# fnothaft/spark-bam

Hardware: AMD Instinct MI355X
Metric: compressed BAM GB/s for compute-splits + full-check (whole node, 1/2/4/8 GPU) (higher is better)
Workload: dtype u8

## Files before the change

### spark-bam_amd/csrc/sbam_api.cpp

```cpp
#include "../../include/sbam.h"

#include <algorithm>
#include <cstdarg>
#include <cstdio>
#include <cstdlib>
#include <cstring>
#include <map>
#include <string>
#include <vector>

#include "sbam_deflate_core.h"
#include "sbam_internal.h"
#include "sbam_layout.h"
#include "sbam_tag_core.h"

using namespace sbam;
using namespace sbam_layout;

namespace {

#define HIPTRY(expr)                 \
  do {                               \
    hipError_t e_ = (expr);          \
    if (e_ != hipSuccess) return e_; \
// ... 184 lines not shown
  DevBuf<int64_t> d_tokbase;
  DevBuf<int32_t> d_slow;
  DevBuf<unsigned int> d_icnt;
  int64_t inflate_slow = -1;
  DevBuf<uint32_t> d_crc, d_crcst;
  int64_t crc_b0 = -1, crc_b1 = -1;
  bool verify_crc = false;
  int32_t nref = -1;
  DevBuf<int64_t> d_lens;
  std::vector<int64_t> h_lens;
  sbam_pos header_end{0, 0, 0};
  int64_t header_x = -1;
  DevBuf<unsigned long long> d_bitmap;
  int64_t bm_x0 = 0, bm_x1 = 0;
  int32_t bm_R = -1;
  bool bm_valid = false;
  bool bm_list = false;
  int64_t plist_n = 0;
  DevBuf<int32_t> d_ccnt;
  DevBuf<int32_t> d_tcnt;
  DevBuf<int64_t> d_coff2, d_plist, d_pfb;
  DevBuf<uint8_t> d_pok;
  DevBuf<unsigned long long> d_nfb;
  DevBuf<int64_t> d_sx, d_se, d_sn, d_sb;
  int32_t rp_tried = 0, rp_proved = 0;
  int64_t rp_missing = -1, rp_failed = -1;
  bool rp_fetch = false;
  DevBuf<int64_t> d_roff;
  DevBuf<uint8_t> d_rcols;
  RecordColumnsDev rcols{};
  int64_t n_loaded = -1;
  DevBuf<uint8_t> d_foff, d_fdata;
  sbam_record_fields fdev{};
  int64_t f_i0 = 0, f_n = -1;
  sbam_record_field_totals f_tot{};
  DevBuf<uint8_t> d_tcell, d_toff, d_tdata;
  sbam_record_tags tdev{};
  int64_t t_i0 = 0, t_n = -1;
  int32_t t_nq = 0;
  bool t_bytes[SBAM_MAX_TAGS] = {};
  sbam_record_tag_totals t_tot{};
  bool loaded_all = false;
  DevBuf<int32_t> d_iend;
  DevBuf<uint32_t> d_ibin;
  DevBuf<int64_t> d_iheads, d_iintv;
  DevBuf<uint8_t> d_istat;
// ... 17 lines not shown
  std::string path = "<bytes>";
};

namespace {

int set_err(sbam_ctx *c, int code, const char *fmt, ...) {
  c->err.code = code;
  va_list ap;
  va_start(ap, fmt);
  vsnprintf(c->err.message, sizeof(c->err.message), fmt, ap);
  va_end(ap);
  return code;
}

#define HIPCHK(ctx, expr)                                                                     \
  do {                                                                                        \
    hipError_t e_ = (expr);                                                                   \
    if (e_ != hipSuccess) return set_err(ctx, SBAM_ERR_HIP, "%s: %s", #expr, hipGetErrorString(e_)); \
  } while (0)

struct Timer {
  sbam_ctx *c;
  std::pair<hipEvent_t, hipEvent_t> *e = nullptr;
  Timer(sbam_ctx *c_, const char *name) : c(c_) {
    if (!c) return;
    auto it = c->ev.find(name);
    if (it == c->ev.end()) {
      std::pair<hipEvent_t, hipEvent_t> p;
      (void)hipEventCreate(&p.first);
      (void)hipEventCreate(&p.second);
      it = c->ev.emplace(name, p).first;
    }
    e = &it->second;
    (void)hipEventRecord(e->first, c->stream);
  }
  ~Timer() { if (c) (void)hipEventRecord(e->second, c->stream); }
};

#define SMALL(c, word) ((c)->d_small.get() + offsetof(Scratch, word) / 8)
#define USMALL(c, word) reinterpret_cast<unsigned long long *>(SMALL(c, word))

template <class F>
hipError_t carve(DevBuf<uint8_t> &buf, bool *grew, F &&layout) {
  Carve size(nullptr);
  layout(size);
  HIPTRY(buf.ensure(size.bytes(), grew));
  Carve k(buf.get());
  layout(k);
  return hipSuccess;
}

StreamView view(sbam_ctx *c) {
  return StreamView{c->d_u, c->L, c->d_lens, c->nref, (c->base + c->D >= c->file_size) ? 1 : 0};
}

void set_bitmap(sbam_ctx *c, int64_t x0, int64_t x1, int32_t R, bool list_form) {
  c->bm_x0 = x0 & ~(int64_t)63;
  c->bm_x1 = x1;
  c->bm_R = R;
// ... 225 lines not shown
  c->file_size = file_size;
  HIPCHK(c, hipSetDevice(device));
  HIPCHK(c, hipStreamCreateWithFlags(&c->stream, hipStreamNonBlocking));
  HIPCHK(c, c->d_comp.ensure((size_t)len + kCompPad));
  HIPCHK(c, hipMemsetAsync(c->d_comp + len, 0, kCompPad, c->stream));
  if (len) HIPCHK(c, hipMemcpyAsync(c->d_comp, data, (size_t)len, hipMemcpyHostToDevice, c->stream));
  HIPCHK(c, c->d_small.ensure(sizeof(Scratch) / 8));
  HIPCHK(c, carve(c->d_counts, nullptr, count_words<CountsDev>));
  HIPCHK(c, hipStreamSynchronize(c->stream));
  return SBAM_OK;
}

void sbam_close(sbam_ctx *c) {
  if (!c) return;
  (void)hipSetDevice(c->device);
  if (c->stream) (void)hipStreamSynchronize(c->stream);
  if (c->blk.copy_stream) (void)hipStreamSynchronize(c->blk.copy_stream);
  for (auto &kv : c->ev) {
    (void)hipEventDestroy(kv.second.first);
    (void)hipEventDestroy(kv.second.second);
  }
  for (hipEvent_t e : c->load_ev)
    if (e) (void)hipEventDestroy(e);
  c->blk.destroy();
  if (c->stream) (void)hipStreamDestroy(c->stream);
  delete c;
}

const sbam_error *sbam_last_error(const sbam_ctx *c) { return c ? &c->err : nullptr; }

int sbam_set_path(sbam_ctx *c, const char *path) {
  if (!c || !path) return SBAM_ERR_ARG;
  c->path = path;
  return SBAM_OK;
}

int sbam_load(sbam_ctx *c, const uint8_t *data, int64_t len, int64_t base_offset, int64_t file_size) {
  if (!c || (!data && len > 0) || len < 0 || base_offset < 0 || file_size < base_offset + len) return SBAM_ERR_ARG;
  HIPCHK(c, hipSetDevice(c->device));
  HIPCHK(c, hipStreamSynchronize(c->stream));
  HIPCHK(c, c->d_comp.ensure((size_t)len + kCompPad));
  HIPCHK(c, hipMemsetAsync(c->d_comp + len, 0, kCompPad, c->stream));
  constexpr int64_t kPiece = 8ll << 20;
  constexpr int kInFlight = 3;
  for (hipEvent_t &e : c->load_ev)
    if (!e) HIPCHK(c, hipEventCreateWithFlags(&e, hipEventDisableTiming));
// ... 31 lines not shown
  HIPCHK(c, ensure_inflate(c, ubytes, n_blocks, &grew));
  HIPCHK(c, ensure_check(c, 0, ubytes, &grew));
  if (n_records > 0) {
    const size_t n = (size_t)(n_records + n_records / 8 + 4096);
    HIPCHK(c, ensure_chain_list(c, n, &grew));
    HIPCHK(c, ensure_record_columns(c, n, &grew));
  }
  if (grew && any_stage_ran(c)) return sbam_reset(c);
  return SBAM_OK;
}

int sbam_reset(sbam_ctx *c) {
  if (!c) return SBAM_ERR_ARG;
  const hipError_t e = drop_from(c, kCandidates);
  c->err = sbam_error{};
  HIPCHK(c, e);
  return SBAM_OK;
}

double sbam_last_kernel_ms(sbam_ctx *c, const char *kernel) {
  if (!std::strcmp(kernel, "record_tags")) {
    const double walk = sbam_last_kernel_ms(c, "record_tag_walk"), bytes = sbam_last_kernel_ms(c, "record_tag_bytes");
    return walk < 0 ? -1.0 : walk + (bytes < 0 ? 0.0 : bytes);
  }
  auto it = c->ev.find(kernel);
  if (it == c->ev.end()) return -1.0;
  (void)hipEventSynchronize(it->second.second);
  float ms = -1.f;
  if (hipEventElapsedTime(&ms, it->second.first, it->second.second) != hipSuccess) return -1.0;
  return ms;
}

static int scan_candidates(sbam_ctx *c) {
  if (c->ncand >= 0) return SBAM_OK;
  Timer t(c, "scan");
  const int64_t nchunks = scan_chunks(c->D);
  HIPCHK(c, ensure_scan(c, c->D));
  HIPCHK(c, launch_scan_slots(c->d_comp, c->D, c->d_cc, nchunks, c->d_slots, SMALL(c, scan_overflow), c->stream));
  HIPCHK(c, launch_scan_sums(c->d_cc, c->d_coff, nchunks, 1, SMALL(c, scan_total), c->stream));
  int64_t tot_ovf[2] = {0, 0};
  HIPCHK(c, hipMemcpyAsync(tot_ovf, SMALL(c, scan_total), 2 * sizeof(int64_t), hipMemcpyDeviceToHost, c->stream));
  HIPCHK(c, hipStreamSynchronize(c->stream));
  const int64_t total = tot_ovf[0];
  HIPCHK(c, c->d_cand.ensure(total));
  if (tot_ovf[1] == 0) {
    HIPCHK(c, launch_scan_compact(c->d_slots, c->d_cc, c->d_coff, nchunks, c->d_cand, c->stream));
// ... 489 lines not shown

static hipError_t run_chains(sbam_ctx *c, int64_t x0, int64_t x1, int32_t R, int32_t by_key, CountsDev cd,
                             bool *list_form, const int32_t *tile_pass0) {
  const int64_t nch = chain_list_chunks(x0, x1);
  const int64_t cap = (x1 - x0) / 32 + 4096;
  HIPTRY(c->d_ccnt.ensure((size_t)std::max<int64_t>(nch, 1)));
  HIPTRY(c->d_coff2.ensure((size_t)nch + 1));
  ChainScratch cs{c->d_ccnt, c->d_coff2, nullptr, nullptr, nullptr, nullptr};
  HIPTRY(launch_chain_list_build(x0, x1, c->d_bitmap, cs, tile_pass0, c->stream));
  int64_t total = 0;
  HIPTRY(hipMemcpyAsync(&total, c->d_coff2 + nch, 8, hipMemcpyDeviceToHost, c->stream));
  HIPTRY(hipStreamSynchronize(c->stream));
  *list_form = total <= cap;
  if (!*list_form) return launch_check_full_chains(view(c), x0, x1, R, by_key, cd, c->d_bitmap, c->stream);
  HIPTRY(ensure_chain_list(c, (size_t)std::max<int64_t>(total, 1)));
  cs.list = c->d_plist;
  cs.ok = c->d_pok;
  cs.fb = c->d_pfb;
  cs.n_fb = c->d_nfb;
  c->plist_n = total;
  return launch_chain_list_run(view(c), x0, x1, R, by_key, cd, c->d_bitmap, cs, c->stream);
}

int sbam_check_full_counts(sbam_ctx *c, int64_t x0, int64_t x1, int32_t R, int32_t by_key, sbam_counts *out,
                           uint64_t *bitmap) {
  if (!c || !out) return SBAM_ERR_ARG;
  int rc = check_range_args(c, x0, x1, R);
  if (rc) return rc;
  HIPCHK(c, hipSetDevice(c->device));
  HIPCHK(c, drop_from(c, kBitmap));
  HIPCHK(c, ensure_check(c, x0, x1));
  Carve k(c->d_counts.get());
  CountsDev cd = count_words<CountsDev>(k);
  cd.tile_pass0 = c->d_tcnt;
  const size_t words = cd.totals + SBAM_NUM_FLAGS - cd.counts;
  HIPCHK(c, hipMemsetAsync(cd.counts, 0, words * 8, c->stream));
  bool tiles = false, list_form = false;
  {
    Timer t(c, "check_full");
    {
      Timer t0(c, "check_pass0");
      HIPCHK(c, launch_check_full_counts(view(c), x0, x1, R, by_key, cd, c->d_bitmap, c->stream, &tiles));
    }
    Timer t1(c, "check_chains");
    HIPCHK(c, run_chains(c, x0, x1, R, by_key, cd, &list_form, tiles ? c->d_tcnt.get() : nullptr));
  }
  std::vector<unsigned long long> hw(words);
  HIPCHK(c, hipMemcpyAsync(hw.data(), cd.counts, words * 8, hipMemcpyDeviceToHost, c->stream));
  HIPCHK(c, hipStreamSynchronize(c->stream));
  if (bitmap) {
    int rc2 = copy_bitmap_out(c, x0, x1, bitmap);
    if (rc2) return rc2;
  }
  memset(out, 0, sizeof(*out));
  Carve hk(hw.data());
  const CountsDev h = count_words<CountsDev>(hk);
  std::memcpy(out->counts, h.counts, sizeof(out->counts));
  std::memcpy(out->positions, h.positions, sizeof(out->positions));
  std::memcpy(out->reads_before_error, h.rbe, sizeof(out->reads_before_error));
  std::memcpy(out->pair_hist, h.pair, sizeof(out->pair_hist));
  std::memcpy(out->totals, h.totals, sizeof(out->totals));
  out->n_positions = x1 - x0;
  out->n_success = (int64_t)h.scalars[1];
  out->n_too_few_fixed = (int64_t)h.scalars[2];
  out->n_halo = (int64_t)h.scalars[3];
  set_bitmap(c, x0, x1, R, list_form);
  if (out->n_halo) {
    c->err.actual = out->n_halo;
    return set_err(c, SBAM_ERR_HALO, "%lld positions need bytes past the shard", (long long)out->n_halo);
  }
  return SBAM_OK;
}
// ... 1010 lines not shown
```

### spark-bam_amd/csrc/sbam_check.hip

```cpp
#include <algorithm>
#include <atomic>
#include <type_traits>

#include "sbam_device.h"
#include "sbam_internal.h"

namespace sbam {

constexpr uint32_t W_SUCC = 0x80000000u, W_HALO = 0x00800000u;
constexpr uint32_t W_PASS0 = 0x40000000u;
constexpr uint32_t W_NONE = 0xffffffffu;
constexpr int kCheckThreads = 256;
constexpr int kTile = 8192;
constexpr int kHalo = 768;
constexpr int kWin = kTile + kHalo;
constexpr int kOpcWords = kWin / 128 + 4;
constexpr int kNameWords = kWin / 32 + 4;
constexpr int kLdsLens = 4096;
constexpr int kCheckWgs = 4, kCheckWgsInt = 5, kCheckWgsBits = 5;
constexpr int kFlushTiles = 7;
static_assert(kWin % 16 == 0, "window");
static_assert((kTile / (4 * kCheckThreads)) % 2 == 0, "groups pair up within a tile (add4_paired)");

SB_DEV uint64_t shfl_xor64(uint64_t v, int m) {
  const uint32_t lo = __shfl_xor((int)(uint32_t)v, m, 64), hi = __shfl_xor((int)(uint32_t)(v >> 32), m, 64);
  return ((uint64_t)hi << 32) | lo;
}

// ... 212 lines not shown
  if (cd.counts) {
    for (int o = 32; o >= 1; o >>= 1) n_succ += __shfl_xor((int)n_succ, o, 64);
    if (lane == 0 && n_succ) atomicAdd(&cd.scalars[1], (unsigned long long)n_succ);
  }
}

__global__ __launch_bounds__(256) void k_p0_count(const unsigned long long *__restrict__ bitmap, int64_t nwords,
                                                  int32_t *__restrict__ chunk_cnt) {
  const int64_t cb = (int64_t)blockIdx.x * kChainWords + threadIdx.x;
  uint32_t c = 0;
#pragma unroll
  for (int j = 0; j < kChainWordsPerThread; j++) {
    const int64_t w = cb + 256 * j;
    c += w < nwords ? (uint32_t)__popcll(bitmap[w]) : 0u;
  }
  c = wave_sum(c);
  __shared__ uint32_t s_c[4];
  if (lane_id() == 0) s_c[threadIdx.x >> 6] = c;
  __syncthreads();
  if (threadIdx.x == 0) chunk_cnt[blockIdx.x] = (int32_t)(s_c[0] + s_c[1] + s_c[2] + s_c[3]);
}

__global__ __launch_bounds__(256) void k_p0_count_tiles(const int32_t *__restrict__ tile_pass0, int64_t ntiles,
                                                        int64_t nch, int32_t *__restrict__ chunk_cnt) {
  const int64_t ch = (int64_t)blockIdx.x * blockDim.x + threadIdx.x;
  if (ch >= nch) return;
  const int64_t t0 = ch * 16, t1 = min(t0 + 16, ntiles);
  int32_t c = 0;
  for (int64_t i = 4 * t0; i < 4 * t1; i++) c += tile_pass0[i];
  chunk_cnt[ch] = c;
}

__global__ __launch_bounds__(256) void k_p0_list(const unsigned long long *__restrict__ bitmap, int64_t nwords,
                                                 int64_t x0a, const int64_t *__restrict__ chunk_off,
                                                 int64_t *__restrict__ list) {
  static_assert(kChainWordsPerThread == 8, "k_p0_list: 8-word runs");
  constexpr int kRow = kChainWordsPerThread + 1;
  __shared__ unsigned long long s_cw[256 * kRow];
  const int64_t cb = (int64_t)blockIdx.x * kChainWords;
#pragma unroll
  for (int j = 0; j < kChainWordsPerThread; j++) {
    const int i = (int)threadIdx.x + 256 * j;
    s_cw[(i >> 3) * kRow + (i & 7)] = cb + i < nwords ? bitmap[cb + i] : 0ull;
  }
  __syncthreads();
  const int64_t w0 = cb + (int64_t)threadIdx.x * kChainWordsPerThread;
  unsigned long long cw[kChainWordsPerThread];
  uint32_t mine = 0;
#pragma unroll
  for (int j = 0; j < kChainWordsPerThread; j++) {
    cw[j] = s_cw[threadIdx.x * kRow + j];
    mine += (uint32_t)__popcll(cw[j]);
  }
  __shared__ uint32_t s_w[4];
  uint32_t total;
  int64_t idx = chunk_off[blockIdx.x] + block_incl_scan<uint32_t, 256>(mine, total, s_w) - mine;
#pragma unroll
  for (int j = 0; j < kChainWordsPerThread; j++)
    for (unsigned long long m = cw[j]; m; m &= m - 1) list[idx++] = x0a + ((w0 + j) << 6) + __builtin_ctzll(m);
}

__global__ __launch_bounds__(256) void k_p0_links(StreamView sv, const int64_t *__restrict__ list,
                                                  const int64_t *__restrict__ n_ptr, int64_t x1,
                                                  uint8_t *__restrict__ ok) {
  const int64_t n = *n_ptr;
  for (int64_t i = (int64_t)blockIdx.x * blockDim.x + threadIdx.x; i < n; i += (int64_t)gridDim.x * blockDim.x) {
    const int64_t p = list[i];
    const int32_t bs = g_i32(sv.u, p);
    const int32_t lrn = sv.u[p + 12];
    const int32_t nc = (int32_t)((uint32_t)sv.u[p + 16] | ((uint32_t)sv.u[p + 17] << 8));
    const int64_t c_end = p + 36 + (lrn >= 2 ? lrn : 0) + 4 * (int64_t)nc;
    const int64_t nxt = p + 4 + (int64_t)bs;
    const bool link = i + 1 < n ? list[i + 1] == nxt : (nxt >= x1 && nxt <= sv.L);
    ok[i] = (link && nxt >= c_end) ? 1 : 0;
  }
}

__global__ __launch_bounds__(256) void k_p0_fast(const int64_t *__restrict__ list, const int64_t *__restrict__ n_ptr,
                                                 const uint8_t *__restrict__ ok, int R, CountsDev cd,
                                                 int64_t *__restrict__ fb, unsigned long long *__restrict__ n_fb) {
  const int64_t n = *n_ptr;
  uint32_t n_succ = 0, n_gap = 0;
  for (int64_t i = (int64_t)blockIdx.x * blockDim.x + threadIdx.x; i < n; i += (int64_t)gridDim.x * blockDim.x) {
    bool succ = i + (R - 1) <= n - 1 || R <= 1;
    for (int k = 0; succ && k < R - 1; k++) succ = ok[i + k] != 0;
    if (succ) n_succ++;
    else fb[atomicAdd(n_fb, 1ull)] = list[i];
    n_gap += !ok[i] ? 1u : 0u;
  }
  if (__ballot(n_gap != 0)) {
    n_gap = wave_sum(n_gap);
    if (lane_id() == 0) atomicAdd(&n_fb[1], (unsigned long long)n_gap);
  }
  if (cd.counts) {
    n_succ = wave_sum(n_succ);
    if (lane_id() == 0 && n_succ) atomicAdd(&cd.scalars[1], (unsigned long long)n_succ);
  }
}

__global__ __launch_bounds__(256) void k_p0_fast16(const int64_t *__restrict__ list, const int64_t *__restrict__ n_ptr,
                                                   const uint8_t *__restrict__ ok, int R, CountsDev cd,
                                                   int64_t *__restrict__ fb, unsigned long long *__restrict__ n_fb) {
  const int64_t n = *n_ptr;
  const uint32_t need = (1u << (R - 1)) - 1u;
  uint32_t n_succ = 0, n_gap = 0;
  auto nib = [](uint32_t w) { return (((w & 0x01010101u) * 0x00204081u) >> 21) & 0xfu; };
  for (int64_t i0 = 16 * ((int64_t)blockIdx.x * blockDim.x + threadIdx.x); i0 < n;
       i0 += 16 * (int64_t)gridDim.x * blockDim.x) {
    uint32_t m = 0;
    if (i0 + 24 <= n) {
      const uint4 a = *reinterpret_cast<const uint4 *>(ok + i0);
      const uint2 b = *reinterpret_cast<const uint2 *>(ok + i0 + 16);
      m = nib(a.x) | nib(a.y) << 4 | nib(a.z) << 8 | nib(a.w) << 12 | nib(b.x) << 16 | nib(b.y) << 20;
    } else {
      for (int k = 0; k < 24 && i0 + k < n; k++) m |= (ok[i0 + k] != 0 ? 1u : 0u) << k;
    }
#pragma unroll
    for (int j = 0; j < 16; j++) {
      const int64_t i = i0 + j;
      if (i < n) {
        const bool succ = i + (R - 1) <= n - 1 && ((m >> j) & need) == need;
        if (succ) n_succ++;
        else fb[atomicAdd(n_fb, 1ull)] = list[i];
        n_gap += !((m >> j) & 1u) ? 1u : 0u;
      }
    }
// ... 1337 lines not shown
      hipLaunchKernelGGL(k_check_bits, dim3(bits_grid(ni, shmem)), dim3(kCheckThreads), shmem, s, sv, x0, R, cd,
                         bitmap, tlo, thi);
    }
    if (nt > ni)
      hipLaunchKernelGGL((k_check<MODE_COUNTS, 2>), dim3(check_grid(nt - ni)), dim3(kCheckThreads), 0, s, sv, x0, x1,
                         R, cd, bitmap, nullptr, tlo, thi);
  } else {
    hipLaunchKernelGGL((k_check<MODE_COUNTS, 0>), dim3(check_grid(ntiles_of(x0, x1))), dim3(kCheckThreads), 0, s, sv,
                       x0, x1, R, cd, bitmap, nullptr, (int64_t)0, (int64_t)0);
  }
  return hipGetLastError();
}
hipError_t launch_check_full_chains(StreamView sv, int64_t x0, int64_t x1, int32_t R, int32_t by_key, CountsDev cd,
                                    unsigned long long *bitmap, hipStream_t s) {
  if (x1 <= x0) return hipSuccess;
  hipLaunchKernelGGL(k_chains, dim3(chain_grid(x0, x1)), dim3(256), 0, s, sv, x0, x1, R, bitmap, cd, by_key, nullptr);
  return hipGetLastError();
}
int64_t chain_list_chunks(int64_t x0, int64_t x1) {
  const int64_t words = (x1 - (x0 & ~(int64_t)63) + 63) >> 6;
  return (words + kChainWords - 1) / kChainWords;
}
static_assert(kChainWords * 64 == 16 * kTile, "a chain chunk is 16 record-0 tiles");
hipError_t launch_chain_list_build(int64_t x0, int64_t x1, const unsigned long long *bitmap, const ChainScratch &cs,
                                   const int32_t *tile_pass0, hipStream_t s) {
  const int64_t x0a = x0 & ~(int64_t)63, nwords = (x1 - x0a + 63) >> 6, nch = chain_list_chunks(x0, x1);
  if (nch <= 0) return hipSuccess;
  if (tile_pass0)
    hipLaunchKernelGGL(k_p0_count_tiles, dim3((unsigned)((nch + 255) / 256)), dim3(256), 0, s, tile_pass0,
                       ntiles_of(x0, x1), nch, cs.chunk_cnt);
  else
    hipLaunchKernelGGL(k_p0_count, dim3((unsigned)nch), dim3(256), 0, s, bitmap, nwords, cs.chunk_cnt);
  return launch_scan_sums(cs.chunk_cnt, cs.chunk_off, nch, 1, cs.chunk_off + nch, s);
}
hipError_t launch_chain_list_run(StreamView sv, int64_t x0, int64_t x1, int32_t R, int32_t by_key, CountsDev cd,
                                 unsigned long long *bitmap, const ChainScratch &cs, hipStream_t s) {
  const int64_t x0a = x0 & ~(int64_t)63, nwords = (x1 - x0a + 63) >> 6, nch = chain_list_chunks(x0, x1);
  if (nch <= 0) return hipSuccess;
  const int64_t *n_ptr = cs.chunk_off + nch;
  hipLaunchKernelGGL(k_p0_list, dim3((unsigned)nch), dim3(256), 0, s, bitmap, nwords, x0a, cs.chunk_off, cs.list);
  hipLaunchKernelGGL(k_p0_links, dim3(4096), dim3(256), 0, s, sv, cs.list, n_ptr, x1, cs.ok);
  (void)hipMemsetAsync(cs.n_fb, 0, 3 * sizeof(unsigned long long), s);
  if (R >= 2 && R <= 10)
    hipLaunchKernelGGL(k_p0_fast16, dim3(1024), dim3(256), 0, s, cs.list, n_ptr, cs.ok, (int)R, cd, cs.fb, cs.n_fb);
  else
    hipLaunchKernelGGL(k_p0_fast, dim3(4096), dim3(256), 0, s, cs.list, n_ptr, cs.ok, (int)R, cd, cs.fb, cs.n_fb);
  hipLaunchKernelGGL(k_p0_fallback, dim3(1024), dim3(256), 0, s, sv, x0a, x1, (int)R, bitmap, cd, (int)by_key, cs.fb,
                     cs.n_fb);
  return hipGetLastError();
}
hipError_t launch_check_eager_pass0(StreamView sv, int64_t x0, int64_t x1, int32_t R, unsigned long long *bitmap,
                                    hipStream_t s) {
  if (x1 <= x0) return hipSuccess;
  if (R == 0) {
    launch_split_check<MODE_EAGER>(sv, x0, x1, R, CountsDev{}, bitmap, s);
    return hipGetLastError();
  }
  int64_t tlo, thi;
  interior_tiles(sv, x0, x1, &tlo, &thi);
  const int64_t nt = ntiles_of(x0, x1), ni = thi - tlo;
  if (ni > 0) {
    const int64_t g = std::max<int64_t>(1, std::min<int64_t>((ni + 10 * kEwWaves - 1) / (10 * kEwWaves), 131072));
    hipLaunchKernelGGL(k_eager_wave, dim3((unsigned)g), dim3(64 * kEwWaves), 0, s, sv, x0, (int)R, bitmap, tlo, thi);
  }
  if (nt > ni)
    hipLaunchKernelGGL((k_check<MODE_EAGER, 2>), dim3(check_grid(nt - ni)), dim3(kCheckThreads), 0, s, sv, x0, x1, R,
                       CountsDev{}, bitmap, nullptr, tlo, thi);
  return hipGetLastError();
}
hipError_t launch_check_words(StreamView sv, int64_t x0, int64_t x1, int32_t R, uint32_t *words,
                              unsigned long long *bitmap, hipStream_t s) {
// ... 28 lines not shown
```

### spark-bam_amd/csrc/sbam_internal.h

```cpp
#pragma once
#include <hip/hip_runtime.h>
#include <cstdlib>
#include <stdint.h>

namespace sbam {

struct Candidate {
  int64_t pos;
  int32_t hsize;
  int32_t csize;
  int32_t isize;
  int32_t flags;
};
enum : int32_t { CAND_ISIZE = 1, CAND_EMPTY = 2 };

struct BlockTable {
  const int64_t *start;
  const int32_t *hsize;
  const int32_t *csize;
  const int32_t *usize;
  const int64_t *uoff;
  int64_t n;
};

// ... 89 lines not shown
hipError_t launch_first_error(const int32_t *status, int64_t n, unsigned long long *first_err, hipStream_t s);
hipError_t launch_lower_bound(const Candidate *c, int64_t n, int64_t q, int64_t *out, hipStream_t s);
hipError_t launch_block_crc(const uint8_t *comp, int64_t D, const uint8_t *u, int64_t L, BlockTable bt, int64_t b0,
                            int64_t b1, uint32_t *crc, uint32_t *stored, unsigned long long *n_bad,
                            unsigned long long *first_bad, hipStream_t s);
hipError_t launch_check_full_counts(StreamView sv, int64_t x0, int64_t x1, int32_t R, int32_t by_key, CountsDev cd,
                                    unsigned long long *bitmap, hipStream_t s, bool *tiles_counted);
int64_t check_tiles(int64_t x0, int64_t x1);
hipError_t launch_check_full_chains(StreamView sv, int64_t x0, int64_t x1, int32_t R, int32_t by_key, CountsDev cd,
                                    unsigned long long *bitmap, hipStream_t s);
struct ChainScratch {
  int32_t *chunk_cnt;
  int64_t *chunk_off;
  int64_t *list;
  uint8_t *ok;
  int64_t *fb;
  unsigned long long *n_fb;
};
int64_t chain_list_chunks(int64_t x0, int64_t x1);
hipError_t launch_chain_list_build(int64_t x0, int64_t x1, const unsigned long long *bitmap, const ChainScratch &cs,
                                   const int32_t *tile_pass0, hipStream_t s);
hipError_t launch_chain_list_run(StreamView sv, int64_t x0, int64_t x1, int32_t R, int32_t by_key, CountsDev cd,
                                 unsigned long long *bitmap, const ChainScratch &cs, hipStream_t s);
hipError_t launch_check_eager_pass0(StreamView sv, int64_t x0, int64_t x1, int32_t R, unsigned long long *bitmap,
                                    hipStream_t s);
hipError_t launch_check_words(StreamView sv, int64_t x0, int64_t x1, int32_t R, uint32_t *words,
                              unsigned long long *bitmap, hipStream_t s);
hipError_t launch_find_record_starts(StreamView sv, const int64_t *x0, int64_t n, int32_t R, int64_t max_read_size,
                                     const unsigned long long *bitmap, int64_t bitmap_x0, int64_t bitmap_x1,
                                     int64_t *out, hipStream_t s);
hipError_t launch_record_counts(StreamView sv, const int64_t *x0, const int64_t *x_end, int64_t n, int64_t *counts,
                                hipStream_t s);
hipError_t launch_record_offsets(StreamView sv, int64_t x0, int64_t x_end, int64_t *offsets, int64_t cap,
                                 int64_t *n_out, hipStream_t s);
hipError_t launch_chain_proof(const uint8_t *u, int64_t L, const unsigned long long *bm, int64_t xa, int64_t X0,
                              int64_t X1, int32_t *fail, const unsigned long long *exact, hipStream_t s);
hipError_t launch_split_popcounts(const unsigned long long *bm, int64_t xa, const int64_t *xs, const int64_t *xe,
                                  int64_t n, int64_t *counts, int32_t *fail, const int64_t *list, int64_t nlist,
                                  const unsigned long long *exact, hipStream_t s);
hipError_t launch_split_offsets(const unsigned long long *bm, int64_t xa, const int64_t *xs, const int64_t *xe,
                                const int64_t *base, int64_t n, int64_t *out, hipStream_t s);
hipError_t launch_record_walk(const uint8_t *u, int64_t L, const int64_t *xs, const int64_t *xe, const int64_t *base,
                              int64_t n, int64_t *out, hipStream_t s);
hipError_t launch_record_spans(const uint8_t *u, int64_t L, const int64_t *offs, int64_t n, int32_t *ref_id,
                               int32_t *start, int32_t *end, hipStream_t s);
hipError_t launch_record_columns(const uint8_t *u, const int64_t *offs, int64_t n, const int64_t *bstart,
// ... 147 lines not shown
```

### spark-bam_amd/csrc/sbam_layout.h

```cpp
#pragma once
#include <cstddef>
#include <cstdint>

#include "../../include/sbam.h"

namespace sbam_layout {

typedef unsigned long long u64;

struct Carve {
  explicit Carve(void *base) : base_(static_cast<uint8_t *>(base)) {}
  template <class T>
  T *take(size_t n, size_t align = 256) {
    at_ = up(at_, align);
    T *p = base_ ? reinterpret_cast<T *>(base_ + at_) : nullptr;
    at_ += n * sizeof(T);
    return p;
  }
  int32_t *i32(size_t n, size_t a = 256) { return take<int32_t>(n, a); }
  int64_t *i64(size_t n, size_t a = 256) { return take<int64_t>(n, a); }
  u64 *w64(size_t n, size_t a = 256) { return take<u64>(n, a); }
  size_t bytes() const { return up(at_, 256); }
  static size_t up(size_t b, size_t a = 256) { return (b + a - 1) & ~(a - 1); }
  uint8_t *base_;
// ... 40 lines not shown
template <class R>
R index_words(Carve &k, size_t nref) {
  return R{k.w64(4), k.w64(nref, 8), k.w64(nref, 8), k.w64(nref, 8), k.w64(nref, 8), k.w64(nref, 8)};
}

struct WriteSel { int64_t *len, *cnt; size_t stride; int64_t *src, *bsum, *tot; };
inline WriteSel write_sel(Carve &k, size_t n, size_t nblk) {
  return {k.i64(n + 2), k.i64(n + 2, 8), n + 2, k.i64(n + 1, 8), k.i64(2 * nblk, 8), k.i64(2, 8)};
}

struct WriteSizes { int64_t *tsz, *bsum, *tot; u64 *n_stored; };
inline WriteSizes write_sizes(Carve &k, size_t batch, size_t nblk) {
  return {k.i64(batch + 1), k.i64(nblk, 8), k.i64(1, 8), k.w64(1, 8)};
}
struct WriteCols { int32_t *pay, *stored, *csize, *usize; };
inline WriteCols write_cols(Carve &k, size_t nb) { return {k.i32(nb), k.i32(nb, 4), k.i32(nb, 4), k.i32(nb, 4)}; }

template <class R>
R count_words(Carve &k) {
  constexpr size_t K = SBAM_NUM_KEYS, F = SBAM_NUM_FLAGS, N = SBAM_MAX_READS_TO_CHECK + 1;
  return R{k.w64(K * F), k.w64(K, 8), k.w64(K * N, 8), k.w64(F * F, 8), k.w64(4, 8), k.w64(F, 8)};
}

}
```

Before: 86.32.

## Slab the full check to overlap pass0 tiles with chain list building on a second stream

Splits the interior tiles of the full check into slabs aligned to chain chunks. Each slab's pass0 bit kernel runs on the main stream while the chain count, scan, list and link kernels for earlier slabs run on a separate non-blocking stream, joined by events before a single decide step. It adds a wave-sized list kernel and a capped list with a fallback to the old chain path when the guessed capacity overflows, and it fetches the counts together with the list total in one sync. The cost is extra streams, events and small launches, plus a fallback path that reruns the chains.

```diff
diff --git a/spark-bam_amd/csrc/sbam_api.cpp b/spark-bam_amd/csrc/sbam_api.cpp
--- a/spark-bam_amd/csrc/sbam_api.cpp
+++ b/spark-bam_amd/csrc/sbam_api.cpp
@@ -230,6 +230,11 @@
   DevBuf<int64_t> d_coff2, d_plist, d_pfb;
   DevBuf<uint8_t> d_pok;
   DevBuf<unsigned long long> d_nfb;
+  hipStream_t chain_stream = nullptr;
+  std::vector<hipEvent_t> slab_ev;
+  hipEvent_t chain_join = nullptr;
+  DevBuf<uint8_t> d_cslab;
+  int slab_n = 0;
   DevBuf<int64_t> d_sx, d_se, d_sn, d_sb;
   int32_t rp_tried = 0, rp_proved = 0;
   int64_t rp_missing = -1, rp_failed = -1;
@@ -293,8 +298,10 @@
 struct Timer {
   sbam_ctx *c;
   std::pair<hipEvent_t, hipEvent_t> *e = nullptr;
-  Timer(sbam_ctx *c_, const char *name) : c(c_) {
+  hipStream_t s = nullptr;
+  Timer(sbam_ctx *c_, const std::string &name, hipStream_t on = nullptr) : c(c_) {
     if (!c) return;
+    s = on ? on : c->stream;
     auto it = c->ev.find(name);
     if (it == c->ev.end()) {
       std::pair<hipEvent_t, hipEvent_t> p;
@@ -303,9 +310,9 @@
       it = c->ev.emplace(name, p).first;
     }
     e = &it->second;
-    (void)hipEventRecord(e->first, c->stream);
-  }
-  ~Timer() { if (c) (void)hipEventRecord(e->second, c->stream); }
+    (void)hipEventRecord(e->first, s);
+  }
+  ~Timer() { if (c) (void)hipEventRecord(e->second, s); }
 };
 
 #define SMALL(c, word) ((c)->d_small.get() + offsetof(Scratch, word) / 8)
@@ -577,6 +584,10 @@
   }
   for (hipEvent_t e : c->load_ev)
     if (e) (void)hipEventDestroy(e);
+  if (c->chain_stream) (void)hipStreamSynchronize(c->chain_stream);
+  for (hipEvent_t e : c->slab_ev) (void)hipEventDestroy(e);
+  if (c->chain_join) (void)hipEventDestroy(c->chain_join);
+  if (c->chain_stream) (void)hipStreamDestroy(c->chain_stream);
   c->blk.destroy();
   if (c->stream) (void)hipStreamDestroy(c->stream);
   delete c;
@@ -654,6 +665,16 @@
   if (!std::strcmp(kernel, "record_tags")) {
     const double walk = sbam_last_kernel_ms(c, "record_tag_walk"), bytes = sbam_last_kernel_ms(c, "record_tag_bytes");
     return walk < 0 ? -1.0 : walk + (bytes < 0 ? 0.0 : bytes);
+  }
+  if (!std::strcmp(kernel, "check_slabs")) return (double)c->slab_n;
+  const bool p0 = !std::strcmp(kernel, "check_pass0"), ch = !std::strcmp(kernel, "check_chains");
+  if (c->slab_n > 0 && (p0 || ch)) {
+    double sum = ch ? sbam_last_kernel_ms(c, "check_chains#decide") : 0.0;
+    for (int s = 0; s < c->slab_n && sum >= 0; s++) {
+      const double ms = sbam_last_kernel_ms(c, (std::string(kernel) + "#" + std::to_string(s)).c_str());
+      sum = ms < 0 ? -1.0 : sum + ms;
+    }
+    return sum;
   }
   auto it = c->ev.find(kernel);
   if (it == c->ev.end()) return -1.0;
@@ -1189,6 +1210,60 @@
   return launch_chain_list_run(view(c), x0, x1, R, by_key, cd, c->d_bitmap, cs, c->stream);
 }
 
+static int64_t env_i64(const char *name, int64_t dflt) {
+  const char *e = std::getenv(name);
+  return e && *e ? std::atoll(e) : dflt;
+}
+static CheckSlabs slabs_of(sbam_ctx *c, int64_t x0, int64_t x1, int32_t R, int32_t by_key, int64_t *tlo, int64_t *thi) {
+  if (!check_slabs_apply(view(c), x0, x1, R, by_key, tlo, thi)) return CheckSlabs{};
+  return check_slabs(chain_list_chunks(x0, x1), env_i64("SBAM_CHECK_SLABS", 2), env_i64("SBAM_CHECK_SLAB_TILES", 0));
+}
+static hipError_t ensure_slab_streams(sbam_ctx *c, int n) {
+  if (!c->chain_stream) HIPTRY(hipStreamCreateWithFlags(&c->chain_stream, hipStreamNonBlocking));
+  if (!c->chain_join) HIPTRY(hipEventCreateWithFlags(&c->chain_join, hipEventDisableTiming));
+  while ((int)c->slab_ev.size() < n) {
+    hipEvent_t e = nullptr;
+    HIPTRY(hipEventCreateWithFlags(&e, hipEventDisableTiming));
+    c->slab_ev.push_back(e);
+  }
+  return hipSuccess;
+}
+static hipError_t run_slabbed(sbam_ctx *c, int64_t x0, int64_t x1, int32_t R, CountsDev cd, const CheckSlabs &sl,
+                              int64_t tlo, int64_t thi, int64_t cap, int64_t **n_ptr) {
+  const int64_t nch = chain_list_chunks(x0, x1);
+  HIPTRY(c->d_ccnt.ensure((size_t)nch));
+  HIPTRY(c->d_coff2.ensure((size_t)nch + 1));
+  HIPTRY(ensure_chain_list(c, (size_t)cap));
+  ChainSlabWords w{};
+  HIPTRY(carve(c->d_cslab, nullptr, [&](Carve &k) { w = chain_slab_words(k, (size_t)sl.n); }));
+  HIPTRY(ensure_slab_streams(c, sl.n));
+  const ChainScratch cs{c->d_ccnt, c->d_coff2, c->d_plist, c->d_pok, c->d_pfb, c->d_nfb};
+  const StreamView sv = view(c);
+  Timer t(c, "check_full");
+  HIPTRY(hipMemsetAsync(w.tot, 0, (size_t)(2 * sl.n + 1) * 8, c->stream));
+  HIPTRY(launch_check_boundary_counts(sv, x0, x1, R, cd, c->d_bitmap, c->stream));
+  for (int s = 0; s < sl.n; s++) {
+    int64_t t0, t1;
+    check_slab_tiles(sl, s, tlo, thi, &t0, &t1);
+    {
+      Timer tp(c, "check_pass0#" + std::to_string(s));
+      HIPTRY(launch_check_bits_tiles(sv, x0, R, cd, c->d_bitmap, t0, t1, c->stream));
+    }
+    HIPTRY(hipEventRecord(c->slab_ev[s], c->stream));
+    HIPTRY(hipStreamWaitEvent(c->chain_stream, c->slab_ev[s], 0));
+    Timer tc(c, "check_chains#" + std::to_string(s), c->chain_stream);
+    const bool last = s == sl.n - 1;
+    const int link_grid = last ? 4096 : 512;
+    HIPTRY(launch_chain_slab(sv, x0, x1, c->d_bitmap, cs, c->d_tcnt, sl.chunk[s], sl.chunk[s + 1], w.tot + s, w.run + s,
+                             link_grid, last, cap, c->chain_stream));
+  }
+  HIPTRY(hipEventRecord(c->chain_join, c->chain_stream));
+  HIPTRY(hipStreamWaitEvent(c->stream, c->chain_join, 0));
+  *n_ptr = w.run + sl.n;
+  Timer td(c, "check_chains#decide");
+  return launch_chain_slabs_decide(sv, x0, x1, R, 0, cd, c->d_bitmap, cs, *n_ptr, cap, c->stream);
+}
+
 int sbam_check_full_counts(sbam_ctx *c, int64_t x0, int64_t x1, int32_t R, int32_t by_key, sbam_counts *out,
                            uint64_t *bitmap) {
   if (!c || !out) return SBAM_ERR_ARG;
@@ -1202,8 +1277,27 @@
   cd.tile_pass0 = c->d_tcnt;
   const size_t words = cd.totals + SBAM_NUM_FLAGS - cd.counts;
   HIPCHK(c, hipMemsetAsync(cd.counts, 0, words * 8, c->stream));
-  bool tiles = false, list_form = false;
-  {
+  bool tiles = false, list_form = false, have_counts = false;
+  int64_t tlo = 0, thi = 0, total = 0;
+  const CheckSlabs sl = slabs_of(c, x0, x1, R, by_key, &tlo, &thi);
+  c->slab_n = sl.n > 1 ? sl.n : 0;
+  std::vector<unsigned long long> hw(words);
+  if (c->slab_n) {
+    const size_t have = std::min(c->d_plist.size(), std::min(c->d_pfb.size(), c->d_pok.size()));
+    int64_t cap = (int64_t)(have ? have : chain_list_guess(x1 - x0));
+    cap = std::max<int64_t>(1, env_i64("SBAM_CHECK_LIST_CAP", cap));
+    int64_t *n_ptr = nullptr;
+    HIPCHK(c, run_slabbed(c, x0, x1, R, cd, sl, tlo, thi, cap, &n_ptr));
+    HIPCHK(c, hipMemcpyAsync(&total, n_ptr, 8, hipMemcpyDeviceToHost, c->stream));
+    HIPCHK(c, hipMemcpyAsync(hw.data(), cd.counts, words * 8, hipMemcpyDeviceToHost, c->stream));
+    HIPCHK(c, hipStreamSynchronize(c->stream));
+    list_form = have_counts = total <= cap;
+    c->plist_n = total;
+    if (!list_form) {
+      Timer t1(c, "check_chains#decide");
+      HIPCHK(c, run_chains(c, x0, x1, R, by_key, cd, &list_form, c->d_tcnt.get()));
+    }
+  } else {
     Timer t(c, "check_full");
     {
       Timer t0(c, "check_pass0");
@@ -1212,9 +1306,10 @@
     Timer t1(c, "check_chains");
     HIPCHK(c, run_chains(c, x0, x1, R, by_key, cd, &list_form, tiles ? c->d_tcnt.get() : nullptr));
   }
-  std::vector<unsigned long long> hw(words);
-  HIPCHK(c, hipMemcpyAsync(hw.data(), cd.counts, words * 8, hipMemcpyDeviceToHost, c->stream));
-  HIPCHK(c, hipStreamSynchronize(c->stream));
+  if (!have_counts) {
+    HIPCHK(c, hipMemcpyAsync(hw.data(), cd.counts, words * 8, hipMemcpyDeviceToHost, c->stream));
+    HIPCHK(c, hipStreamSynchronize(c->stream));
+  }
   if (bitmap) {
     int rc2 = copy_bitmap_out(c, x0, x1, bitmap);
     if (rc2) return rc2;
diff --git a/spark-bam_amd/csrc/sbam_check.hip b/spark-bam_amd/csrc/sbam_check.hip
--- a/spark-bam_amd/csrc/sbam_check.hip
+++ b/spark-bam_amd/csrc/sbam_check.hip
@@ -4,6 +4,7 @@
 
 #include "sbam_device.h"
 #include "sbam_internal.h"
+#include "sbam_layout.h"
 
 namespace sbam {
 
@@ -262,8 +263,8 @@
 }
 
 __global__ __launch_bounds__(256) void k_p0_count_tiles(const int32_t *__restrict__ tile_pass0, int64_t ntiles,
-                                                        int64_t nch, int32_t *__restrict__ chunk_cnt) {
-  const int64_t ch = (int64_t)blockIdx.x * blockDim.x + threadIdx.x;
+                                                        int64_t c0, int64_t nch, int32_t *__restrict__ chunk_cnt) {
+  const int64_t ch = c0 + (int64_t)blockIdx.x * blockDim.x + threadIdx.x;
   if (ch >= nch) return;
   const int64_t t0 = ch * 16, t1 = min(t0 + 16, ntiles);
   int32_t c = 0;
@@ -271,13 +272,37 @@
   chunk_cnt[ch] = c;
 }
 
+__global__ __launch_bounds__(256) void k_p0_slab_scan(const int32_t *__restrict__ cnt, int64_t *__restrict__ off,
+                                                      int64_t n, int64_t *__restrict__ total_out) {
+  __shared__ int64_t ws[4];
+  const int64_t per = (n + 255) / 256;
+  const int64_t b = min((int64_t)threadIdx.x * per, n), e = min(b + per, n);
+  int64_t sum = 0;
+  for (int64_t i = b; i < e; i++) sum += cnt[i];
+  int64_t total;
+  int64_t run = block_incl_scan<int64_t, 256>(sum, total, ws) - sum;
+  for (int64_t i = b; i < e; i++) {
+    off[i] = run;
+    run += cnt[i];
+  }
+  if (threadIdx.x == 0) *total_out = total;
+}
+
+struct ListSlab {
+  int64_t c0 = 0;
+  int64_t *run = nullptr;
+  const int64_t *tot = nullptr;
+  int64_t cap = INT64_MAX;
+};
 __global__ __launch_bounds__(256) void k_p0_list(const unsigned long long *__restrict__ bitmap, int64_t nwords,
                                                  int64_t x0a, const int64_t *__restrict__ chunk_off,
-                                                 int64_t *__restrict__ list) {
+                                                 int64_t *__restrict__ list, ListSlab sl) {
   static_assert(kChainWordsPerThread == 8, "k_p0_list: 8-word runs");
   constexpr int kRow = kChainWordsPerThread + 1;
   __shared__ unsigned long long s_cw[256 * kRow];
-  const int64_t cb = (int64_t)blockIdx.x * kChainWords;
+  const int64_t ch = sl.c0 + blockIdx.x, cb = ch * kChainWords;
+  const int64_t first = sl.run ? sl.run[0] : 0;
+  if (sl.run && blockIdx.x == 0 && threadIdx.x == 0) sl.run[1] = first + *sl.tot;
 #pragma unroll
   for (int j = 0; j < kChainWordsPerThread; j++) {
     const int i = (int)threadIdx.x + 256 * j;
@@ -294,17 +319,64 @@
   }
   __shared__ uint32_t s_w[4];
   uint32_t total;
-  int64_t idx = chunk_off[blockIdx.x] + block_incl_scan<uint32_t, 256>(mine, total, s_w) - mine;
+  int64_t idx = first + chunk_off[ch] + block_incl_scan<uint32_t, 256>(mine, total, s_w) - mine;
 #pragma unroll
   for (int j = 0; j < kChainWordsPerThread; j++)
-    for (unsigned long long m = cw[j]; m; m &= m - 1) list[idx++] = x0a + ((w0 + j) << 6) + __builtin_ctzll(m);
+    for (unsigned long long m = cw[j]; m; m &= m - 1, idx++)
+      if (idx < sl.cap) list[idx] = x0a + ((w0 + j) << 6) + __builtin_ctzll(m);
+}
+
+constexpr int kListWavePer = 2;
+constexpr int kListWaveRound = 64 * kListWavePer;
+static_assert(kChainWords % kListWaveRound == 0, "k_p0_list_wave: whole rounds");
+__global__ __launch_bounds__(64) __attribute__((amdgpu_num_vgpr(16))) void k_p0_list_wave(const unsigned long long *__restrict__ bitmap, int64_t nwords,
+                                                     int64_t x0a, const int64_t *__restrict__ chunk_off,
+                                                     int64_t *__restrict__ list, ListSlab sl) {
+  constexpr int kRow = kListWavePer + 1;
+  __shared__ unsigned long long s_cw[64 * kRow];
+  const int lane = (int)threadIdx.x;
+  const int64_t ch = sl.c0 + blockIdx.x, cb = ch * kChainWords;
+  const int64_t first = sl.run[0];
+  if (blockIdx.x == 0 && lane == 0) sl.run[1] = first + *sl.tot;
+  int64_t at = first + chunk_off[ch];
+#pragma unroll 1
+  for (int r = 0; r < kChainWords / kListWaveRound; r++) {
+    const int64_t rb = cb + (int64_t)r * kListWaveRound;
+#pragma unroll
+    for (int j = 0; j < kListWavePer; j++) {
+      const int i = lane + 64 * j;
+      s_cw[(i / kListWavePer) * kRow + (i % kListWavePer)] = rb + i < nwords ? bitmap[rb + i] : 0ull;
+    }
+    __syncthreads();
+    unsigned long long cw[kListWavePer];
+    uint32_t mine = 0;
+#pragma unroll
+    for (int j = 0; j < kListWavePer; j++) {
+      cw[j] = s_cw[lane * kRow + j];
+      mine += (uint32_t)__popcll(cw[j]);
+    }
+    __syncthreads();
+    const uint32_t incl = wave_incl_scan(mine);
+    uint32_t k = incl - mine;
+    const int64_t base = x0a + (rb << 6);
+    const uint32_t b0 = (uint32_t)(lane * kListWavePer) << 6;
+#pragma unroll
+    for (int j = 0; j < kListWavePer; j++)
+      for (unsigned long long m = cw[j]; m; m &= m - 1, k++)
+        if (at + k < sl.cap) list[at + k] = base + (b0 + (uint32_t)(j << 6) + (uint32_t)__builtin_ctzll(m));
+    at += (uint32_t)__shfl((int)incl, 63, 64);
+  }
 }
 
 __global__ __launch_bounds__(256) void k_p0_links(StreamView sv, const int64_t *__restrict__ list,
-                                                  const int64_t *__restrict__ n_ptr, int64_t x1,
+                                                  const int64_t *__restrict__ lo_ptr,
+                                                  const int64_t *__restrict__ n_ptr, int last, int64_t cap, int64_t x1,
                                                   uint8_t *__restrict__ ok) {
-  const int64_t n = *n_ptr;
-  for (int64_t i = (int64_t)blockIdx.x * blockDim.x + threadIdx.x; i < n; i += (int64_t)gridDim.x * blockDim.x) {
+  const int64_t n = *n_ptr, lo = lo_ptr ? *lo_ptr : 0;
+  if (n > cap) return;
+  const int64_t i0 = lo > 0 ? lo - 1 : 0, i1 = last ? n : n - 1;
+  for (int64_t i = i0 + (int64_t)blockIdx.x * blockDim.x + threadIdx.x; i < i1;
+       i += (int64_t)gridDim.x * blockDim.x) {
     const int64_t p = list[i];
     const int32_t bs = g_i32(sv.u, p);
     const int32_t lrn = sv.u[p + 12];
@@ -318,8 +390,10 @@
 
 __global__ __launch_bounds__(256) void k_p0_fast(const int64_t *__restrict__ list, const int64_t *__restrict__ n_ptr,
                                                  const uint8_t *__restrict__ ok, int R, CountsDev cd,
-                                                 int64_t *__restrict__ fb, unsigned long long *__restrict__ n_fb) {
+                                                 int64_t *__restrict__ fb, unsigned long long *__restrict__ n_fb,
+                                                 int64_t cap) {
   const int64_t n = *n_ptr;
+  if (n > cap) return;
   uint32_t n_succ = 0, n_gap = 0;
   for (int64_t i = (int64_t)blockIdx.x * blockDim.x + threadIdx.x; i < n; i += (int64_t)gridDim.x * blockDim.x) {
     bool succ = i + (R - 1) <= n - 1 || R <= 1;
@@ -340,8 +414,10 @@
 
 __global__ __launch_bounds__(256) void k_p0_fast16(const int64_t *__restrict__ list, const int64_t *__restrict__ n_ptr,
                                                    const uint8_t *__restrict__ ok, int R, CountsDev cd,
-                                                   int64_t *__restrict__ fb, unsigned long long *__restrict__ n_fb) {
+                                                   int64_t *__restrict__ fb, unsigned long long *__restrict__ n_fb,
+                                                   int64_t cap) {
   const int64_t n = *n_ptr;
+  if (n > cap) return;
   const uint32_t need = (1u << (R - 1)) - 1u;
   uint32_t n_succ = 0, n_gap = 0;
   auto nib = [](uint32_t w) { return (((w & 0x01010101u) * 0x00204081u) >> 21) & 0xfu; };
@@ -1725,31 +1801,95 @@
   return (words + kChainWords - 1) / kChainWords;
 }
 static_assert(kChainWords * 64 == 16 * kTile, "a chain chunk is 16 record-0 tiles");
+static_assert(sbam_layout::kChunkTiles * kTile == kChainWords * 64, "check_slabs cuts at chain chunks");
 hipError_t launch_chain_list_build(int64_t x0, int64_t x1, const unsigned long long *bitmap, const ChainScratch &cs,
                                    const int32_t *tile_pass0, hipStream_t s) {
   const int64_t x0a = x0 & ~(int64_t)63, nwords = (x1 - x0a + 63) >> 6, nch = chain_list_chunks(x0, x1);
   if (nch <= 0) return hipSuccess;
   if (tile_pass0)
     hipLaunchKernelGGL(k_p0_count_tiles, dim3((unsigned)((nch + 255) / 256)), dim3(256), 0, s, tile_pass0,
-                       ntiles_of(x0, x1), nch, cs.chunk_cnt);
+                       ntiles_of(x0, x1), (int64_t)0, nch, cs.chunk_cnt);
   else
     hipLaunchKernelGGL(k_p0_count, dim3((unsigned)nch), dim3(256), 0, s, bitmap, nwords, cs.chunk_cnt);
   return launch_scan_sums(cs.chunk_cnt, cs.chunk_off, nch, 1, cs.chunk_off + nch, s);
+}
+static void launch_chain_decide(StreamView sv, int64_t x0, int64_t x1, int32_t R, int32_t by_key, CountsDev cd,
+                                unsigned long long *bitmap, const ChainScratch &cs, const int64_t *n_ptr, int64_t cap,
+                                hipStream_t s) {
+  const int64_t x0a = x0 & ~(int64_t)63;
+  if (R >= 2 && R <= 10)
+    hipLaunchKernelGGL(k_p0_fast16, dim3(1024), dim3(256), 0, s, cs.list, n_ptr, cs.ok, (int)R, cd, cs.fb, cs.n_fb,
+                       cap);
+  else
+    hipLaunchKernelGGL(k_p0_fast, dim3(4096), dim3(256), 0, s, cs.list, n_ptr, cs.ok, (int)R, cd, cs.fb, cs.n_fb, cap);
+  hipLaunchKernelGGL(k_p0_fallback, dim3(1024), dim3(256), 0, s, sv, x0a, x1, (int)R, bitmap, cd, (int)by_key, cs.fb,
+                     cs.n_fb);
 }
 hipError_t launch_chain_list_run(StreamView sv, int64_t x0, int64_t x1, int32_t R, int32_t by_key, CountsDev cd,
                                  unsigned long long *bitmap, const ChainScratch &cs, hipStream_t s) {
   const int64_t x0a = x0 & ~(int64_t)63, nwords = (x1 - x0a + 63) >> 6, nch = chain_list_chunks(x0, x1);
   if (nch <= 0) return hipSuccess;
   const int64_t *n_ptr = cs.chunk_off + nch;
-  hipLaunchKernelGGL(k_p0_list, dim3((unsigned)nch), dim3(256), 0, s, bitmap, nwords, x0a, cs.chunk_off, cs.list);
-  hipLaunchKernelGGL(k_p0_links, dim3(4096), dim3(256), 0, s, sv, cs.list, n_ptr, x1, cs.ok);
+  hipLaunchKernelGGL(k_p0_list, dim3((unsigned)nch), dim3(256), 0, s, bitmap, nwords, x0a, cs.chunk_off, cs.list,
+                     ListSlab{});
+  hipLaunchKernelGGL(k_p0_links, dim3(4096), dim3(256), 0, s, sv, cs.list, (const int64_t *)nullptr, n_ptr, 1,
+                     INT64_MAX, x1, cs.ok);
   (void)hipMemsetAsync(cs.n_fb, 0, 3 * sizeof(unsigned long long), s);
-  if (R >= 2 && R <= 10)
-    hipLaunchKernelGGL(k_p0_fast16, dim3(1024), dim3(256), 0, s, cs.list, n_ptr, cs.ok, (int)R, cd, cs.fb, cs.n_fb);
-  else
-    hipLaunchKernelGGL(k_p0_fast, dim3(4096), dim3(256), 0, s, cs.list, n_ptr, cs.ok, (int)R, cd, cs.fb, cs.n_fb);
-  hipLaunchKernelGGL(k_p0_fallback, dim3(1024), dim3(256), 0, s, sv, x0a, x1, (int)R, bitmap, cd, (int)by_key, cs.fb,
-                     cs.n_fb);
+  launch_chain_decide(sv, x0, x1, R, by_key, cd, bitmap, cs, n_ptr, INT64_MAX, s);
+  return hipGetLastError();
+}
+
+bool check_slabs_apply(const StreamView &sv, int64_t x0, int64_t x1, int32_t R, int32_t by_key, int64_t *tlo,
+                       int64_t *thi) {
+  if (x1 <= x0 || by_key || R <= 0) return false;
+  interior_tiles(sv, x0, x1, tlo, thi);
+  return *thi > *tlo;
+}
+hipError_t launch_check_boundary_counts(StreamView sv, int64_t x0, int64_t x1, int32_t R, CountsDev cd,
+                                        unsigned long long *bitmap, hipStream_t s) {
+  int64_t tlo, thi;
+  interior_tiles(sv, x0, x1, &tlo, &thi);
+  const int64_t nt = ntiles_of(x0, x1), ni = thi - tlo;
+  if (nt > ni)
+    hipLaunchKernelGGL((k_check<MODE_COUNTS, 2>), dim3(check_grid(nt - ni)), dim3(kCheckThreads), 0, s, sv, x0, x1, R,
+                       cd, bitmap, nullptr, tlo, thi);
+  return hipGetLastError();
+}
+hipError_t launch_check_bits_tiles(StreamView sv, int64_t x0, int32_t R, CountsDev cd, unsigned long long *bitmap,
+                                   int64_t t0, int64_t t1, hipStream_t s) {
+  if (t1 <= t0) return hipSuccess;
+  const size_t shmem = (sv.nref <= kLdsLens ? (size_t)sv.nref + 1 : 1) * sizeof(int32_t);
+  hipLaunchKernelGGL(k_check_bits, dim3(bits_grid(t1 - t0, shmem)), dim3(kCheckThreads), shmem, s, sv, x0, R, cd,
+                     bitmap, t0, t1);
+  return hipGetLastError();
+}
+hipError_t launch_chain_slab(StreamView sv, int64_t x0, int64_t x1, const unsigned long long *bitmap,
+                             const ChainScratch &cs, const int32_t *tile_pass0, int64_t c0, int64_t c1, int64_t *tot,
+                             int64_t *run, int link_grid, bool last, int64_t cap, hipStream_t s) {
+  const int64_t x0a = x0 & ~(int64_t)63, nwords = (x1 - x0a + 63) >> 6, n = c1 - c0;
+  if (n <= 0) return hipSuccess;
+  hipLaunchKernelGGL(k_p0_count_tiles, dim3((unsigned)((n + 255) / 256)), dim3(256), 0, s, tile_pass0,
+                     ntiles_of(x0, x1), c0, c1, cs.chunk_cnt);
+  ListSlab sl;
+  sl.c0 = c0, sl.run = run, sl.tot = tot, sl.cap = cap;
+  if (last) {
+    const hipError_t e = launch_scan_sums(cs.chunk_cnt + c0, cs.chunk_off + c0, n, 1, tot, s);
+    if (e != hipSuccess) return e;
+    hipLaunchKernelGGL(k_p0_list, dim3((unsigned)n), dim3(256), 0, s, bitmap, nwords, x0a, cs.chunk_off, cs.list, sl);
+  } else {
+    hipLaunchKernelGGL(k_p0_slab_scan, dim3(1), dim3(256), 0, s, cs.chunk_cnt + c0, cs.chunk_off + c0, n, tot);
+    hipLaunchKernelGGL(k_p0_list_wave, dim3((unsigned)n), dim3(64), 0, s, bitmap, nwords, x0a, cs.chunk_off, cs.list,
+                       sl);
+  }
+  hipLaunchKernelGGL(k_p0_links, dim3((unsigned)link_grid), dim3(256), 0, s, sv, cs.list, (const int64_t *)run,
+                     (const int64_t *)(run + 1), last ? 1 : 0, cap, x1, cs.ok);
+  return hipGetLastError();
+}
+hipError_t launch_chain_slabs_decide(StreamView sv, int64_t x0, int64_t x1, int32_t R, int32_t by_key, CountsDev cd,
+                                     unsigned long long *bitmap, const ChainScratch &cs, const int64_t *n_ptr,
+                                     int64_t cap, hipStream_t s) {
+  (void)hipMemsetAsync(cs.n_fb, 0, 3 * sizeof(unsigned long long), s);
+  launch_chain_decide(sv, x0, x1, R, by_key, cd, bitmap, cs, n_ptr, cap, s);
   return hipGetLastError();
 }
 hipError_t launch_check_eager_pass0(StreamView sv, int64_t x0, int64_t x1, int32_t R, unsigned long long *bitmap,
diff --git a/spark-bam_amd/csrc/sbam_internal.h b/spark-bam_amd/csrc/sbam_internal.h
--- a/spark-bam_amd/csrc/sbam_internal.h
+++ b/spark-bam_amd/csrc/sbam_internal.h
@@ -135,6 +135,18 @@
                                    const int32_t *tile_pass0, hipStream_t s);
 hipError_t launch_chain_list_run(StreamView sv, int64_t x0, int64_t x1, int32_t R, int32_t by_key, CountsDev cd,
                                  unsigned long long *bitmap, const ChainScratch &cs, hipStream_t s);
+bool check_slabs_apply(const StreamView &sv, int64_t x0, int64_t x1, int32_t R, int32_t by_key, int64_t *tlo,
+                       int64_t *thi);
+hipError_t launch_check_boundary_counts(StreamView sv, int64_t x0, int64_t x1, int32_t R, CountsDev cd,
+                                        unsigned long long *bitmap, hipStream_t s);
+hipError_t launch_check_bits_tiles(StreamView sv, int64_t x0, int32_t R, CountsDev cd, unsigned long long *bitmap,
+                                   int64_t t0, int64_t t1, hipStream_t s);
+hipError_t launch_chain_slab(StreamView sv, int64_t x0, int64_t x1, const unsigned long long *bitmap,
+                             const ChainScratch &cs, const int32_t *tile_pass0, int64_t c0, int64_t c1, int64_t *tot,
+                             int64_t *run, int link_grid, bool last, int64_t cap, hipStream_t s);
+hipError_t launch_chain_slabs_decide(StreamView sv, int64_t x0, int64_t x1, int32_t R, int32_t by_key, CountsDev cd,
+                                     unsigned long long *bitmap, const ChainScratch &cs, const int64_t *n_ptr,
+                                     int64_t cap, hipStream_t s);
 hipError_t launch_check_eager_pass0(StreamView sv, int64_t x0, int64_t x1, int32_t R, unsigned long long *bitmap,
                                     hipStream_t s);
 hipError_t launch_check_words(StreamView sv, int64_t x0, int64_t x1, int32_t R, uint32_t *words,
diff --git a/spark-bam_amd/csrc/sbam_layout.h b/spark-bam_amd/csrc/sbam_layout.h
--- a/spark-bam_amd/csrc/sbam_layout.h
+++ b/spark-bam_amd/csrc/sbam_layout.h
@@ -86,4 +86,42 @@
   return R{k.w64(K * F), k.w64(K, 8), k.w64(K * N, 8), k.w64(F * F, 8), k.w64(4, 8), k.w64(F, 8)};
 }
 
+constexpr int64_t kChunkTiles = 16;
+constexpr int kMaxCheckSlabs = 64;
+struct CheckSlabs {
+  int n = 0;
+  int64_t chunk[kMaxCheckSlabs + 1] = {};
+};
+inline CheckSlabs check_slabs(int64_t nch, int64_t want, int64_t len_tiles) {
+  CheckSlabs r;
+  if (nch <= 0) return r;
+  int64_t len;
+  if (len_tiles > 0) {
+    len = len_tiles / kChunkTiles + (len_tiles % kChunkTiles ? 1 : 0);
+  } else {
+    const int64_t w = want < 1 ? 1 : want > kMaxCheckSlabs ? kMaxCheckSlabs : want;
+    const int64_t q = 4 * (w - 1) + 1;
+    len = 4 * nch / q + (4 * nch % q ? 1 : 0);
+  }
+  const int64_t min_len = nch / kMaxCheckSlabs + (nch % kMaxCheckSlabs ? 1 : 0);
+  if (len < min_len) len = min_len;
+  if (len > nch) len = nch;
+  r.n = (int)(nch / len + (nch % len ? 1 : 0));
+  for (int s = 0; s < r.n; s++) r.chunk[s] = s * len;
+  r.chunk[r.n] = nch;
+  return r;
 }
+inline void check_slab_tiles(const CheckSlabs &sl, int s, int64_t tlo, int64_t thi, int64_t *t0, int64_t *t1) {
+  const int64_t a = sl.chunk[s] * kChunkTiles, b = sl.chunk[s + 1] * kChunkTiles;
+  *t0 = a > tlo ? a : tlo;
+  *t1 = b < thi ? b : thi;
+  if (*t1 < *t0) *t1 = *t0;
+}
+struct ChainSlabWords { int64_t *tot, *run; };
+inline ChainSlabWords chain_slab_words(Carve &k, size_t nslab) { return {k.i64(nslab), k.i64(nslab + 1, 8)}; }
+inline size_t chain_list_guess(int64_t positions) {
+  const size_t n = (size_t)(positions < 0 ? 0 : positions) / 200;
+  return n + n / 8 + 4096;
+}
+
+}
```

After: 87.10, median of 6. About the same (+0.9%).
